# wubinzzu/NeuRec

Measured on NVIDIA H100. Metric: triplets/sec, higher is better.
Workload: dtype f32

## Files before the change

### include/neurec_b200.h

```cpp
#ifndef NEUREC_B200_H
#define NEUREC_B200_H

#include <stdint.h>

#ifdef __cplusplus
extern "C" {
#endif

#define NRC_OK 0
#define NRC_E_VALUE (-1)
#define NRC_E_TYPE (-2)
#define NRC_E_NOTIMPL (-3)
#define NRC_E_CUDA (-4)
#define NRC_E_LIMIT (-5)

#define NRC_METRIC_PRECISION 1
#define NRC_METRIC_RECALL 2
#define NRC_METRIC_MAP 3
#define NRC_METRIC_NDCG 4
#define NRC_METRIC_MRR 5

#define NRC_LOSS_BPR 0
#define NRC_LOSS_HINGE 1
#define NRC_LOSS_SQUARE 2
// ... 123 lines not shown
                       uint64_t seed, uint64_t epoch, int32_t batch_size, int64_t first_step,
                       int64_t num_steps, int32_t loss_kind, float reg, int32_t opt_kind,
                       const float* hyper_host, float* adam_pows, float* grad_user,
                       float* grad_item, int32_t* touched_user, int32_t* touched_item,
                       float* slot0_user, float* slot1_user, float* slot0_item, float* slot1_item,
                       int32_t first_stamp, int32_t* ws_users, int32_t* ws_items, void* ws_third,
                       float* step_loss, void* stream);

int nrc_batch_randint_choice(int32_t high, const int64_t* out_indptr, int32_t n_rows,
                             int64_t total_out, int32_t replace, const int64_t* excl_indptr,
                             const int32_t* excl_indices, uint64_t seed, uint64_t stream_id,
                             int32_t* out, void* stream);


int nrc_mf_pairwise_grad(const float* user_table, const float* item_table, int32_t dim,
                         const int32_t* users, const int32_t* pos_items,
                         const int32_t* neg_items, int64_t batch, int32_t loss_kind, float reg,
                         float* grad_user, float* grad_item, int32_t* touched_user,
                         int32_t* touched_item, int32_t stamp, float* loss, void* stream);

int nrc_mf_pointwise_grad(const float* user_table, const float* item_table, int32_t dim,
                          const int32_t* users, const int32_t* items, const float* labels,
                          int64_t batch, int32_t loss_kind, float reg, float* grad_user,
                          float* grad_item, int32_t* touched_user, int32_t* touched_item,
                          int32_t stamp, float* loss, void* stream);

int nrc_opt_apply_rows(int32_t opt_kind, float* var, float* grad, float* slot0, float* slot1,
                       const int32_t* touched, int32_t stamp, int64_t rows, int32_t dim,
                       const float* hyper_host, void* stream);

int nrc_mf_bpr_sgd_fused(float* user_table, float* item_table, int32_t dim, const int32_t* users,
                         const int32_t* pos_items, const int32_t* neg_items, int64_t batch,
                         float lr, float reg, float* loss, void* stream);

int nrc_mf_bpr_sgd_sharded(float* const* user_shards, float* const* item_shards, int32_t world,
                           int32_t self_rank, int64_t users_per_shard, int64_t items_per_shard, int32_t dim,
                           const int32_t* users, const int32_t* pos_items, const int32_t* neg_items,
                           int64_t batch, float lr, float reg, float* loss, void* stream);
int nrc_mf_bpr_sgd_epoch(float* user_table, float* const* item_shards, int32_t world,
                         int32_t self_rank, int64_t items_per_shard, int32_t dim,
                         const int64_t* train_indptr, const int32_t* train_indices,
                         const int32_t* pos_users, const int32_t* pos_items, int64_t n_pos,
                         int32_t num_items, int32_t shuffle, uint64_t seed, uint64_t epoch,
                         int64_t first, int64_t count, float lr, float reg, float* loss,
                         void* stream);

int nrc_mf_bpr_sgd_epoch_hot(float* user_table, float* const* item_shards, int32_t world,
                             int32_t self_rank, int64_t items_per_shard, int32_t dim,
                             const int64_t* train_indptr, const int32_t* train_indices,
                             const int32_t* pos_users, const int32_t* pos_items, int64_t n_pos,
                             int32_t num_items, int32_t shuffle, uint64_t seed, uint64_t epoch,
                             int64_t first, int64_t count, float lr, float reg, float* loss,
                             float* hot, float* hot_delta, int32_t n_hot, void* stream);
int nrc_mf_hot_apply(float* hot, float* hot_delta, int64_t n_floats, void* stream);

int nrc_mf_last_routes(int32_t* out);


int nrc_mf_bpr_lazy_adam_epoch(float* user_table, float* user_m, float* user_v, float* item_table,
                               float* item_m, float* item_v, int32_t dim, const int64_t* train_indptr,
                               const int32_t* train_indices, const int32_t* pos_users,
                               const int32_t* pos_items, int64_t n_pos, int32_t num_items,
                               int32_t shuffle, uint64_t seed, uint64_t epoch, int64_t first,
                               int64_t count, float lr_t, float beta1, float beta2, float eps,
                               float reg, float* loss, void* stream);

int nrc_shard_alloc(int64_t nbytes, void** dev_ptr_out, void* handle64_out);
int nrc_shard_free(void* dev_ptr);

int nrc_enable_peer_access(int32_t peer_device);
int nrc_ipc_export(const void* dev_ptr, void* handle64_out, int64_t* offset_out);
int nrc_ipc_open(const void* handle64, int64_t offset, void** dev_ptr_out);
int nrc_ipc_close(void* dev_ptr, int64_t offset);

int nrc_opt_apply_multi(int32_t opt_kind, int32_t n_vars, float* const* var, float* const* grad,
                        float* const* slot0, float* const* slot1, const int32_t* const* touched,
                        const int64_t* rows, const int32_t* dims, const int32_t* dense_var,
                        int32_t stamp, const float* hyper_host, void* stream);

int nrc_mf_train_epoch(float* user_table, float* item_table, int32_t num_users,
                       int32_t num_items, int32_t dim, const int32_t* users,
                       const int32_t* items, const void* third, int64_t n, int32_t batch_size,
                       int32_t pairwise, int32_t loss_kind, float reg, int32_t opt_kind,
                       const float* lr_t_host, const float* hyper_host, float* grad_user,
                       float* grad_item, int32_t* touched_user, int32_t* touched_item,
                       float* slot0_user, float* slot1_user, float* slot0_item,
                       float* slot1_item, int32_t first_stamp, float* step_loss, void* stream);

int nrc_mf_train_step_host(float* user_table, float* item_table, int32_t num_users,
                           int32_t num_items, int32_t dim, const int32_t* users_host,
                           const int32_t* items_host, const void* third_host, int64_t batch,
                           int32_t pairwise, int32_t loss_kind, float reg, int32_t opt_kind,
                           const float* hyper_host, float* grad_user, float* grad_item,
                           int32_t* touched_user, int32_t* touched_item, float* slot0_user,
                           float* slot1_user, float* slot0_item, float* slot1_item,
                           int32_t stamp, void* staging, float* loss_host, void* stream);


typedef struct nrc_ncf_shape {
    int32_t num_users, num_items;
    int32_t mf_dim, mlp_dim;
    int32_t n_layers;
    int32_t layers[4];
    int32_t n_towers;
} nrc_ncf_shape;

// ... 199 lines not shown
```

### neurec_b200/csrc/train_mf.cu

```cuda
#include <stdlib.h>

#include "common.cuh"
#include "epoch.cuh"
#include "learner.cuh"
#include "mf.cuh"
#include "mf_routes.cuh"
#include "optim.cuh"

namespace nrc {

int32_t g_mf_routes[kMfKernels][kMfFields] = {{-1, -1, -1, -1, -1, -1, -1}, {-1, -1, -1, -1, -1, -1, -1},
                                              {-1, -1, -1, -1, -1, -1, -1}, {-1, -1, -1, -1, -1, -1, -1},
                                              {-1, -1, -1, -1, -1, -1, -1}, {-1, -1, -1, -1, -1, -1, -1}};

template <bool PAIRWISE>
__global__ void __launch_bounds__(256)
mf_grad_kernel(const float* __restrict__ U, const float* __restrict__ V, int D, const int32_t* __restrict__ users,
               const int32_t* __restrict__ items, const int32_t* __restrict__ third, int64_t batch, int loss_kind,
               float reg, float* __restrict__ gU, float* __restrict__ gV, int32_t* __restrict__ tU,
               int32_t* __restrict__ tV, int32_t stamp, float* __restrict__ loss) {
    const int lane = threadIdx.x & 31;
    const int wib = threadIdx.x >> 5;
    const int wpb = blockDim.x >> 5;
    const float inv_b = 1.0f / (float)batch;
// ... 113 lines not shown
    mf_route(kMfSgdIds, dim == 128 ? 4 : dim == 64 ? 2 : 1, sharded, -1, -1, blocks, capped, -1);
    if (dim == 128) { if (sharded) NRC_LAUNCH_SGD(4, true); else NRC_LAUNCH_SGD(4, false); }
    else if (dim == 64) { if (sharded) NRC_LAUNCH_SGD(2, true); else NRC_LAUNCH_SGD(2, false); }
    else { if (sharded) NRC_LAUNCH_SGD(1, true); else NRC_LAUNCH_SGD(1, false); }
#undef NRC_LAUNCH_SGD
    NRC_CUDA_CHECK(cudaGetLastError());
    return NRC_OK;
}


template <int VEC>
constexpr int kSgdTierRows = 8192 / (32 * VEC);
template <int VEC>
constexpr size_t kSgdTierBytes = (size_t)2 * kSgdTierRows<VEC> * 32 * VEC * sizeof(float);

template <int VEC, bool SHARDED>
__device__ __forceinline__ void load_item(const RowShards& V, int32_t id, int nt, const float* s_val, int lane,
                                          float (&v)[VEC]) {
    if (id < nt) {
        ld_vec<VEC>(s_val + id * (32 * VEC) + lane * VEC, v);
    } else {
        bool remote;
        float* upd;
        ld_vec<VEC>(V.row<SHARDED>(id, 32 * VEC, remote, upd) + lane * VEC, v);
    }
}

template <int VEC, bool SHARDED>
__device__ __forceinline__ void update_item(const RowShards& V, int32_t id, int nt, float* s_dlt, int lane,
                                            const float (&d)[VEC]) {
    if (id < nt) {
#pragma unroll
        for (int t = 0; t < VEC; ++t) atomicAdd(s_dlt + id * (32 * VEC) + t * 32 + lane, d[t]);
    } else {
        bool remote;
        float* upd;
        V.row<SHARDED>(id, 32 * VEC, remote, upd);
        red_row<VEC>(upd + lane * VEC, d, remote && V.vec_remote == 0);
    }
}

__device__ __forceinline__ float add_as_red(float x, float d) {
    float r;
    asm("add.rn.ftz.f32 %0, %1, %2;" : "=f"(r) : "f"(x), "f"(d));
    return r;
}

constexpr int64_t kOnceMaxRow = 32;
constexpr int32_t kUserOnce = INT32_MIN;

__device__ __forceinline__ void stream_sample(const EpochSpec& E, int64_t p, int64_t first, int64_t count, bool user_once,
                                              int32_t& u, int32_t& item, int32_t& third) {
    const int64_t idx = feistel_perm(E.perm, p);
    u = __ldg(E.users + idx);
    item = __ldg(E.pos + idx);
    const int64_t beg = __ldg(E.tptr + u), end = __ldg(E.tptr + u + 1);
    third = philox_draw_excluding((uint64_t)(idx * E.neg_num), E.seed, E.stream_id, E.num_items, E.tidx + beg, end - beg);
    if (user_once && end - beg <= kOnceMaxRow) {
        bool alone = true;
#pragma unroll 1
        for (int64_t q = beg; q < end; ++q) {
            if (q == idx) continue;
            const int64_t r = feistel_perm_inv(E.perm, q);
            alone &= (uint64_t)(r - first) >= (uint64_t)count;
        }
        if (alone) u |= kUserOnce;
    }
}

constexpr int kStreamThreads = 768;

template <int VEC, bool SHARDED>
__global__ void __launch_bounds__(kStreamThreads, 1)
mf_bpr_sgd_stream_kernel(float* __restrict__ U_local, const RowShards V, const EpochSpec E, int64_t first,
                         int64_t count, int user_once, float lr, float reg, float* __restrict__ loss) {
    constexpr int D = 32 * VEC, CH = kStreamThreads, T = kSgdTierRows<VEC>;
    constexpr int TPW = 2;
    __shared__ int32_t s_u[CH], s_i[CH], s_j[CH];
    extern __shared__ __align__(16) float s_tier[];
    float* const s_val = s_tier;
    float* const s_dlt = s_tier + T * D;
    const int lane = threadIdx.x & 31, warp = threadIdx.x >> 5;
    const int nt = V.n_hot < T ? V.n_hot : T;
    for (int e = threadIdx.x; e < nt * D / 4; e += blockDim.x) {
        reinterpret_cast<float4*>(s_val)[e] = reinterpret_cast<const float4*>(V.hot)[e];
        reinterpret_cast<float4*>(s_dlt)[e] = make_float4(0.f, 0.f, 0.f, 0.f);
    }
    const int64_t lo = count * blockIdx.x / gridDim.x, hi = count * (blockIdx.x + 1) / gridDim.x;
    float loss_acc = 0.0f;
    for (int64_t c0 = lo; c0 < hi; c0 += CH) {
        const int n = (hi - c0 < CH) ? (int)(hi - c0) : CH;
        if ((int)threadIdx.x < n) {
            int32_t u, i, j;
            stream_sample(E, first + c0 + threadIdx.x, first, count, user_once != 0, u, i, j);
            s_u[threadIdx.x] = u; s_i[threadIdx.x] = i; s_j[threadIdx.x] = j;
        }
        __syncthreads();
        for (int t0 = warp * TPW; t0 < n; t0 += (kStreamThreads / 32) * TPW) {
            float a[TPW][VEC], b[TPW][VEC], c[TPW][VEC];
#pragma unroll
            for (int k = 0; k < TPW; ++k) {
                const int t = (t0 + k < n) ? t0 + k : t0;
                ld_vec<VEC>(U_local + (size_t)(s_u[t] & ~kUserOnce) * D + lane * VEC, a[k]);
                load_item<VEC, SHARDED>(V, s_i[t], nt, s_val, lane, b[k]);
                load_item<VEC, SHARDED>(V, s_j[t], nt, s_val, lane, c[k]);
            }
            float di[TPW], dj[TPW], sq[TPW];
#pragma unroll
            for (int k = 0; k < TPW; ++k) {
                di[k] = 0.f; dj[k] = 0.f; sq[k] = 0.f;
#pragma unroll
                for (int t = 0; t < VEC; ++t) {
                    di[k] = fmaf(a[k][t], b[k][t], di[k]); dj[k] = fmaf(a[k][t], c[k][t], dj[k]);
                    sq[k] += a[k][t] * a[k][t] + b[k][t] * b[k][t] + c[k][t] * c[k][t];
                }
                di[k] = warp_sum(di[k]); dj[k] = warp_sum(dj[k]);
            }
#pragma unroll
            for (int k = 0; k < TPW; ++k) {
                if (t0 + k >= n) break;
                const int t = t0 + k;
                const float x = di[k] - dj[k];
                float l = neg_log_sigmoid(x);
                if (reg != 0.0f) l += reg * 0.5f * warp_sum(sq[k]);
                loss_acc += l;
                const float g = neg_log_sigmoid_grad(x);
                float du[VEC], dvi[VEC], dvj[VEC];
#pragma unroll
                for (int q = 0; q < VEC; ++q) {
                    du[q] = -lr * (g * (b[k][q] - c[k][q]) + reg * a[k][q]);
                    dvi[q] = -lr * (g * a[k][q] + reg * b[k][q]);
                    dvj[q] = -lr * (-g * a[k][q] + reg * c[k][q]);
                }
                const int32_t su = s_u[t];
                float* const pu = U_local + (size_t)(su & ~kUserOnce) * D + lane * VEC;
                if (su & kUserOnce) {
#pragma unroll
                    for (int q = 0; q < VEC; ++q) du[q] = add_as_red(a[k][q], du[q]);
                    st_vec<VEC>(pu, du);
                } else {
                    red_row<VEC>(pu, du, false);
                }
                update_item<VEC, SHARDED>(V, s_i[t], nt, s_dlt, lane, dvi);
                update_item<VEC, SHARDED>(V, s_j[t], nt, s_dlt, lane, dvj);
            }
        }
        __syncthreads();
    }
    __syncthreads();
    for (int e = threadIdx.x; e < nt * 32; e += blockDim.x) {
        const int r = e >> 5, l = e & 31;
        float d[VEC];
        bool any = false;
#pragma unroll
        for (int t = 0; t < VEC; ++t) { d[t] = s_dlt[r * D + t * 32 + l]; any |= d[t] != 0.0f; }
        if (any) red_row<VEC>(V.hot_delta + (size_t)r * D + l * VEC, d, false);
    }
    if (lane == 0 && loss) atomicAdd(loss, loss_acc);
}

template <int VEC, bool SH>
static int launch_stream(float* U_local, const RowShards& SV, const EpochSpec& E, int64_t first, int64_t count,
                         int user_once, float lr, float reg, float* loss, cudaStream_t st) {
    constexpr size_t smem = kSgdTierBytes<VEC>;
    static int64_t grid_cap = 0;
    if (!grid_cap) {
        NRC_CUDA_CHECK(cudaFuncSetAttribute(mf_bpr_sgd_stream_kernel<VEC, SH>, cudaFuncAttributeMaxDynamicSharedMemorySize,
                                            (int)smem));
        int per_sm = 0;
        NRC_CUDA_CHECK(cudaOccupancyMaxActiveBlocksPerMultiprocessor(&per_sm, mf_bpr_sgd_stream_kernel<VEC, SH>, kStreamThreads, smem));
        NRC_REQUIRE(per_sm > 0, NRC_E_CUDA, "mf_bpr_sgd_stream_kernel does not fit on an SM");
        grid_cap = (int64_t)per_sm * sm_count();
    }
    int64_t blocks = (count + kStreamThreads - 1) / kStreamThreads;
    const bool capped = blocks > grid_cap;
    if (blocks > grid_cap) blocks = grid_cap;
    mf_route(kMfSgdCsr, VEC, SH, user_once, SV.n_hot < kSgdTierRows<VEC> ? SV.n_hot : kSgdTierRows<VEC>, blocks, capped,
             -1);
    mf_bpr_sgd_stream_kernel<VEC, SH><<<(unsigned)blocks, kStreamThreads, smem, st>>>(U_local, SV, E, first, count,
                                                                                      user_once, lr, reg, loss);
    NRC_CUDA_CHECK(cudaGetLastError());
    return NRC_OK;
}

static int launch_bpr_sgd_stream(float* U_local, const RowShards& SV, int dim, const EpochSpec& E, int64_t first,
                                 int64_t count, float lr, float reg, float* loss, cudaStream_t st) {
    const bool sharded = SV.rows_per_shard != 0;
    const int user_once = E.pos == E.tidx ? 1 : 0;
#define NRC_STREAM(VEC) (sharded ? launch_stream<VEC, true>(U_local, SV, E, first, count, user_once, lr, reg, loss, st) \
                                 : launch_stream<VEC, false>(U_local, SV, E, first, count, user_once, lr, reg, loss, st))
    if (dim == 128) return NRC_STREAM(4);
    if (dim == 64) return NRC_STREAM(2);
    return NRC_STREAM(1);
#undef NRC_STREAM
}

template <int VEC>
__device__ __forceinline__ void lazy_adam_row(float* var, float* m, float* v, const float (&x)[VEC], float (&mm)[VEC],
                                              float (&vv)[VEC], const float (&g)[VEC], float lr_t, float b1, float b2,
                                              float eps) {
    float out[VEC];
#pragma unroll
    for (int t = 0; t < VEC; ++t) {
        mm[t] = b1 * mm[t] + (1.0f - b1) * g[t];
        vv[t] = b2 * vv[t] + (1.0f - b2) * g[t] * g[t];
        out[t] = x[t] - lr_t * mm[t] / (sqrtf(vv[t]) + eps);
    }
    st_vec<VEC>(m, mm); st_vec<VEC>(v, vv); st_vec<VEC>(var, out);
}

template <int VEC>
__global__ void __launch_bounds__(256, 3)
mf_bpr_lazy_adam_stream_kernel(float* __restrict__ U, float* __restrict__ mU, float* __restrict__ vU, float* __restrict__ V,
                               float* __restrict__ mV, float* __restrict__ vV, const EpochSpec E, int64_t first, int64_t count,
                               float lr_t, float b1, float b2, float eps, float reg, float* __restrict__ loss) {
    constexpr int D = 32 * VEC;
    constexpr int CH = 256;
    __shared__ int32_t s_u[CH], s_i[CH], s_j[CH];
    const int lane = threadIdx.x & 31, warp = threadIdx.x >> 5;
    float loss_acc = 0.0f;
    for (int64_t c0 = (int64_t)blockIdx.x * CH; c0 < count; c0 += (int64_t)gridDim.x * CH) {
        const int n = (count - c0 < CH) ? (int)(count - c0) : CH;
        if ((int)threadIdx.x < n) {
            int32_t u, i, j;
            epoch_sample(E, first + c0 + threadIdx.x, 0, u, i, j);
            s_u[threadIdx.x] = u; s_i[threadIdx.x] = i; s_j[threadIdx.x] = j;
        }
        __syncthreads();
        for (int t = warp; t < n; t += 8) {
            const size_t ou = (size_t)s_u[t] * D + lane * VEC, oi = (size_t)s_i[t] * D + lane * VEC,
                         oj = (size_t)s_j[t] * D + lane * VEC;
            float a[VEC], bi[VEC], bj[VEC], mu[VEC], vu[VEC], mi[VEC], vi[VEC], mj[VEC], vj[VEC];
            ld_vec<VEC>(U + ou, a); ld_vec<VEC>(V + oi, bi); ld_vec<VEC>(V + oj, bj);
            ld_vec<VEC>(mU + ou, mu); ld_vec<VEC>(vU + ou, vu);
            ld_vec<VEC>(mV + oi, mi); ld_vec<VEC>(vV + oi, vi);
            ld_vec<VEC>(mV + oj, mj); ld_vec<VEC>(vV + oj, vj);
            float di = 0.f, dj = 0.f, sq = 0.f;
#pragma unroll
            for (int c = 0; c < VEC; ++c) {
                di = fmaf(a[c], bi[c], di); dj = fmaf(a[c], bj[c], dj);
                sq += a[c] * a[c] + bi[c] * bi[c] + bj[c] * bj[c];
            }
            di = warp_sum(di); dj = warp_sum(dj);
            const float x = di - dj;
            float l = neg_log_sigmoid(x);
            if (reg != 0.0f) l += reg * 0.5f * warp_sum(sq);
            loss_acc += l;
// ... 92 lines not shown
    if (batch <= 0) return NRC_OK;
    RowShards SU{}, SV{};
    for (int r = 0; r < world; ++r) {
        NRC_REQUIRE(user_shards[r] != nullptr && item_shards[r] != nullptr, NRC_E_VALUE, "shard %d is NULL", r);
        SU.base[r] = user_shards[r];
        SV.base[r] = item_shards[r];
    }
    SU.rows_per_shard = (int32_t)users_per_shard;
    SV.rows_per_shard = (int32_t)items_per_shard;
    SU.self = SV.self = self_rank;
    SU.vec_remote = SV.vec_remote = peer_red_mode();
    return launch_bpr_sgd(SU, SV, dim, users, pos_items, neg_items, batch, lr, reg, loss, as_stream(stream));
}

extern "C" int nrc_mf_bpr_sgd_epoch_hot(float* user_table, float* const* item_shards, int32_t world, int32_t self_rank,
                                    int64_t items_per_shard, int32_t dim, const int64_t* train_indptr,
                                    const int32_t* train_indices, const int32_t* pos_users, const int32_t* pos_items,
                                    int64_t n_pos, int32_t num_items, int32_t shuffle, uint64_t seed, uint64_t epoch,
                                    int64_t first, int64_t count, float lr, float reg, float* loss, float* hot, float* hot_delta,
                                    int32_t n_hot, void* stream) {
    NRC_REQUIRE(world >= 1 && world <= 8, NRC_E_LIMIT, "world %d outside [1, 8]", world);
    NRC_REQUIRE(self_rank >= 0 && self_rank < world, NRC_E_VALUE, "self_rank %d outside [0, %d)", self_rank, world);
    NRC_REQUIRE(user_table != nullptr && item_shards != nullptr, NRC_E_VALUE, "table pointers are NULL");
    NRC_REQUIRE(dim == 32 || dim == 64 || dim == 128, NRC_E_LIMIT, "fused SGD supports dim 32, 64, 128 (got %d)", dim);
    NRC_REQUIRE(world == 1 || (items_per_shard > 0 && items_per_shard * world < (1ll << 31) &&
                               items_per_shard * world >= num_items),
                NRC_E_VALUE, "items_per_shard %lld x world %d must cover num_items %d and fit int32",
                (long long)items_per_shard, world, num_items);
    EpochSpec E;
    int rc = epoch_spec_init(E, train_indptr, train_indices, pos_users, pos_items, n_pos, 1, num_items, 1, shuffle, seed,
                             epoch);
    if (rc) return rc;
    NRC_REQUIRE(first >= 0 && count >= 0 && first + count <= n_pos, NRC_E_VALUE,
                "[first, first + count) = [%lld, %lld) outside the epoch's %lld triplets", (long long)first,
                (long long)(first + count), (long long)n_pos);
    if (count == 0) return NRC_OK;
    RowShards SV{};
    for (int r = 0; r < world; ++r) {
        NRC_REQUIRE(item_shards[r] != nullptr, NRC_E_VALUE, "item shard %d is NULL", r);
        SV.base[r] = item_shards[r];
    }
    SV.rows_per_shard = world > 1 ? (int32_t)items_per_shard : 0;
    SV.self = self_rank;
    NRC_REQUIRE(n_hot >= 0 && n_hot <= num_items && (n_hot == 0 || (hot != nullptr && hot_delta != nullptr)), NRC_E_VALUE,
                "n_hot %d needs 0 <= n_hot <= num_items and the replica / delta buffers", n_hot);
    SV.hot = hot; SV.hot_delta = hot_delta; SV.n_hot = n_hot;
    {
        static int vec = -1, force = -1;
        if (vec < 0) vec = peer_red_mode();
        if (force < 0) { const char* e = getenv("NRC_FORCE_REMOTE_PATH"); force = e ? atoi(e) : 0; }
        SV.vec_remote = vec;
        SV.force_remote = force;
    }
    return launch_bpr_sgd_stream(user_table, SV, dim, E, first, count, lr, reg, loss, as_stream(stream));
}

extern "C" int nrc_mf_bpr_sgd_epoch(float* user_table, float* const* item_shards, int32_t world, int32_t self_rank,
                                    int64_t items_per_shard, int32_t dim, const int64_t* train_indptr,
                                    const int32_t* train_indices, const int32_t* pos_users, const int32_t* pos_items,
                                    int64_t n_pos, int32_t num_items, int32_t shuffle, uint64_t seed, uint64_t epoch,
                                    int64_t first, int64_t count, float lr, float reg, float* loss, void* stream) {
    return nrc_mf_bpr_sgd_epoch_hot(user_table, item_shards, world, self_rank, items_per_shard, dim, train_indptr,
                                    train_indices, pos_users, pos_items, n_pos, num_items, shuffle, seed, epoch, first,
                                    count, lr, reg, loss, nullptr, nullptr, 0, stream);
}

namespace nrc {
__global__ void __launch_bounds__(256) hot_apply_kernel(float4* __restrict__ hot, float4* __restrict__ delta, int64_t n4) {
    for (int64_t e = (int64_t)blockIdx.x * blockDim.x + threadIdx.x; e < n4; e += (int64_t)gridDim.x * blockDim.x) {
        float4 h = hot[e];
        const float4 d = delta[e];
        h.x += d.x; h.y += d.y; h.z += d.z; h.w += d.w;
        hot[e] = h;
        delta[e] = make_float4(0.f, 0.f, 0.f, 0.f);
    }
}
}

extern "C" int nrc_mf_hot_apply(float* hot, float* hot_delta, int64_t n_floats, void* stream) {
    NRC_REQUIRE(n_floats >= 0 && (n_floats & 3) == 0, NRC_E_VALUE, "n_floats %lld must be a multiple of 4", (long long)n_floats);
    if (n_floats == 0) return NRC_OK;
    NRC_REQUIRE(hot && hot_delta, NRC_E_VALUE, "replica / delta pointers are NULL");
    int64_t blocks = (n_floats / 4 + 255) / 256;
    const int64_t cap = (int64_t)sm_count() * 8;
    if (blocks > cap) blocks = cap;
    hot_apply_kernel<<<(unsigned)blocks, 256, 0, as_stream(stream)>>>(reinterpret_cast<float4*>(hot),
                                                                      reinterpret_cast<float4*>(hot_delta), n_floats / 4);
    NRC_CUDA_CHECK(cudaGetLastError());
    return NRC_OK;
}

extern "C" int nrc_mf_bpr_lazy_adam_epoch(float* user_table, float* user_m, float* user_v, float* item_table, float* item_m,
                                          float* item_v, int32_t dim, const int64_t* train_indptr,
                                          const int32_t* train_indices, const int32_t* pos_users, const int32_t* pos_items,
                                          int64_t n_pos, int32_t num_items, int32_t shuffle, uint64_t seed, uint64_t epoch,
                                          int64_t first, int64_t count, float lr_t, float beta1, float beta2, float eps,
                                          float reg, float* loss, void* stream) {
    NRC_REQUIRE(dim == 32 || dim == 64 || dim == 128, NRC_E_LIMIT, "lazy Adam supports dim 32, 64, 128 (got %d)", dim);
    NRC_REQUIRE(user_table && user_m && user_v && item_table && item_m && item_v, NRC_E_VALUE, "table / slot pointers are NULL");
    EpochSpec E;
    int rc = epoch_spec_init(E, train_indptr, train_indices, pos_users, pos_items, n_pos, 1, num_items, 1, shuffle, seed,
                             epoch);
    if (rc) return rc;
    NRC_REQUIRE(first >= 0 && count >= 0 && first + count <= n_pos, NRC_E_VALUE,
                "[first, first + count) = [%lld, %lld) outside the epoch's %lld triplets", (long long)first,
                (long long)(first + count), (long long)n_pos);
    if (count == 0) return NRC_OK;
// ... 149 lines not shown
```

Baseline: 850.1 million.

## Split CSR sampling into prefetched side-stream kernel and skip atomics for unique items

Triplet sampling moves out of the SGD stream kernel into a separate sampling kernel that writes u/i/j buffers. It also builds seen/multi bitmaps marking items that occur more than once in the window. The next window is sampled speculatively on a side stream, fenced by fork/join events, so it can overlap the SGD kernel of the current call. Items that appear only once in a window are updated with plain stores instead of reductions, and the user's CSR row bounds are inferred from a vectorised 16-wide load of the users array. The costs are extra buffers, memsets and bitmap atomics, host-side cache state keyed on the window, and a register cap of 64 on the SGD kernel.

```diff
diff --git a/include/neurec_b200.h b/include/neurec_b200.h
--- a/include/neurec_b200.h
+++ b/include/neurec_b200.h
@@ -199,6 +199,7 @@
                              int32_t num_items, int32_t shuffle, uint64_t seed, uint64_t epoch,
                              int64_t first, int64_t count, float lr, float reg, float* loss,
                              float* hot, float* hot_delta, int32_t n_hot, void* stream);
+int nrc_mf_sgd_prefetch(int32_t enable);
 int nrc_mf_hot_apply(float* hot, float* hot_delta, int64_t n_floats, void* stream);
 
 int nrc_mf_last_routes(int32_t* out);
diff --git a/neurec_b200/csrc/train_mf.cu b/neurec_b200/csrc/train_mf.cu
--- a/neurec_b200/csrc/train_mf.cu
+++ b/neurec_b200/csrc/train_mf.cu
@@ -189,9 +189,31 @@
 __device__ __forceinline__ void stream_sample(const EpochSpec& E, int64_t p, int64_t first, int64_t count, bool user_once,
                                               int32_t& u, int32_t& item, int32_t& third) {
     const int64_t idx = feistel_perm(E.perm, p);
-    u = __ldg(E.users + idx);
     item = __ldg(E.pos + idx);
-    const int64_t beg = __ldg(E.tptr + u), end = __ldg(E.tptr + u + 1);
+    int64_t beg = -1, end = -1;
+    const int64_t b0 = idx & ~(int64_t)15;
+    if (user_once && ((uintptr_t)E.users & 63) == 0 && b0 + 16 <= E.n_pos) {
+        int32_t v[16];
+#pragma unroll
+        for (int t = 0; t < 4; ++t) {
+            const int4 q = __ldg(reinterpret_cast<const int4*>(E.users + b0) + t);
+            v[4 * t] = q.x; v[4 * t + 1] = q.y; v[4 * t + 2] = q.z; v[4 * t + 3] = q.w;
+        }
+        const int k = (int)(idx - b0);
+        u = v[0];
+#pragma unroll
+        for (int t = 1; t < 16; ++t) u = t == k ? v[t] : u;
+        int lo = 0, hi = 16;
+#pragma unroll
+        for (int t = 0; t < 16; ++t) {
+            if (t < k && v[t] != u) lo = t + 1;
+            if (t > k && v[t] != u && hi == 16) hi = t;
+        }
+        if ((lo > 0 || b0 == 0) && (hi < 16 || b0 + 16 == E.n_pos)) { beg = b0 + lo; end = b0 + hi; }
+    } else {
+        u = __ldg(E.users + idx);
+    }
+    if (beg < 0) { beg = __ldg(E.tptr + u); end = __ldg(E.tptr + u + 1); }
     third = philox_draw_excluding((uint64_t)(idx * E.neg_num), E.seed, E.stream_id, E.num_items, E.tidx + beg, end - beg);
     if (user_once && end - beg <= kOnceMaxRow) {
         bool alone = true;
@@ -205,12 +227,46 @@
     }
 }
 
+struct SgdIds {
+    int32_t* u;
+    int32_t* i;
+    int32_t* j;
+    uint32_t* seen;
+    uint32_t* multi;
+};
+
+__global__ void __launch_bounds__(256, 8)
+sgd_sample_kernel(const EpochSpec E, int64_t first, int64_t count, int user_once, int32_t n_hot, SgdIds ids) {
+    for (int64_t k = (int64_t)blockIdx.x * blockDim.x + threadIdx.x; k < count; k += (int64_t)gridDim.x * blockDim.x) {
+        int32_t u, i, j;
+        stream_sample(E, first + k, first, count, user_once != 0, u, i, j);
+        ids.u[k] = u; ids.i[k] = i; ids.j[k] = j;
+#pragma unroll
+        for (int r = 0; r < 2; ++r) {
+            const int32_t id = r ? j : i;
+            if (id < n_hot) continue;
+            const uint32_t bit = 1u << (id & 31);
+            if (atomicOr(ids.seen + (id >> 5), bit) & bit) atomicOr(ids.multi + (id >> 5), bit);
+        }
+    }
+}
+
+template <bool SHARDED>
+__device__ __forceinline__ bool item_once(const RowShards& V, const uint32_t* multi, int32_t id) {
+    if constexpr (SHARDED) {
+        return false;
+    } else {
+        if (id < V.n_hot || V.force_remote) return false;
+        return ((__ldg(multi + (id >> 5)) >> (id & 31)) & 1u) == 0;
+    }
+}
+
 constexpr int kStreamThreads = 768;
 
 template <int VEC, bool SHARDED>
-__global__ void __launch_bounds__(kStreamThreads, 1)
-mf_bpr_sgd_stream_kernel(float* __restrict__ U_local, const RowShards V, const EpochSpec E, int64_t first,
-                         int64_t count, int user_once, float lr, float reg, float* __restrict__ loss) {
+__global__ void __maxnreg__(64)
+mf_bpr_sgd_stream_kernel(float* __restrict__ U_local, const RowShards V, const SgdIds ids, int64_t count, float lr,
+                         float reg, float* __restrict__ loss) {
     constexpr int D = 32 * VEC, CH = kStreamThreads, T = kSgdTierRows<VEC>;
     constexpr int TPW = 2;
     __shared__ int32_t s_u[CH], s_i[CH], s_j[CH];
@@ -224,23 +280,29 @@
         reinterpret_cast<float4*>(s_dlt)[e] = make_float4(0.f, 0.f, 0.f, 0.f);
     }
     const int64_t lo = count * blockIdx.x / gridDim.x, hi = count * (blockIdx.x + 1) / gridDim.x;
+    int32_t nu = 0, ni = 0, nj = 0;
+    auto fetch = [&](int64_t c0) {
+        const int64_t k = c0 + threadIdx.x;
+        if (k < hi) { nu = __ldg(ids.u + k); ni = __ldg(ids.i + k); nj = __ldg(ids.j + k); }
+    };
+    fetch(lo);
     float loss_acc = 0.0f;
     for (int64_t c0 = lo; c0 < hi; c0 += CH) {
         const int n = (hi - c0 < CH) ? (int)(hi - c0) : CH;
-        if ((int)threadIdx.x < n) {
-            int32_t u, i, j;
-            stream_sample(E, first + c0 + threadIdx.x, first, count, user_once != 0, u, i, j);
-            s_u[threadIdx.x] = u; s_i[threadIdx.x] = i; s_j[threadIdx.x] = j;
-        }
+        if ((int)threadIdx.x < n) { s_u[threadIdx.x] = nu; s_i[threadIdx.x] = ni; s_j[threadIdx.x] = nj; }
         __syncthreads();
+        fetch(c0 + CH);
         for (int t0 = warp * TPW; t0 < n; t0 += (kStreamThreads / 32) * TPW) {
             float a[TPW][VEC], b[TPW][VEC], c[TPW][VEC];
+            bool oi[TPW], oj[TPW];
 #pragma unroll
             for (int k = 0; k < TPW; ++k) {
                 const int t = (t0 + k < n) ? t0 + k : t0;
                 ld_vec<VEC>(U_local + (size_t)(s_u[t] & ~kUserOnce) * D + lane * VEC, a[k]);
                 load_item<VEC, SHARDED>(V, s_i[t], nt, s_val, lane, b[k]);
                 load_item<VEC, SHARDED>(V, s_j[t], nt, s_val, lane, c[k]);
+                oi[k] = item_once<SHARDED>(V, ids.multi, s_i[t]);
+                oj[k] = item_once<SHARDED>(V, ids.multi, s_j[t]);
             }
             float di[TPW], dj[TPW], sq[TPW];
 #pragma unroll
@@ -278,8 +340,20 @@
                 } else {
                     red_row<VEC>(pu, du, false);
                 }
-                update_item<VEC, SHARDED>(V, s_i[t], nt, s_dlt, lane, dvi);
-                update_item<VEC, SHARDED>(V, s_j[t], nt, s_dlt, lane, dvj);
+                if (oi[k]) {
+#pragma unroll
+                    for (int q = 0; q < VEC; ++q) dvi[q] = add_as_red(b[k][q], dvi[q]);
+                    st_vec<VEC>(V.base[0] + (size_t)s_i[t] * D + lane * VEC, dvi);
+                } else {
+                    update_item<VEC, SHARDED>(V, s_i[t], nt, s_dlt, lane, dvi);
+                }
+                if (oj[k]) {
+#pragma unroll
+                    for (int q = 0; q < VEC; ++q) dvj[q] = add_as_red(c[k][q], dvj[q]);
+                    st_vec<VEC>(V.base[0] + (size_t)s_j[t] * D + lane * VEC, dvj);
+                } else {
+                    update_item<VEC, SHARDED>(V, s_j[t], nt, s_dlt, lane, dvj);
+                }
             }
         }
         __syncthreads();
@@ -296,9 +370,89 @@
     if (lane == 0 && loss) atomicAdd(loss, loss_acc);
 }
 
+struct SgdWindow {
+    const int64_t* tptr;
+    const int32_t* tidx;
+    const int32_t* users;
+    const int32_t* pos;
+    int64_t n_pos, first, count;
+    uint64_t seed, epoch;
+    int32_t num_items, shuffle, n_hot;
+    bool operator==(const SgdWindow& o) const {
+        return tptr == o.tptr && tidx == o.tidx && users == o.users && pos == o.pos && n_pos == o.n_pos &&
+               first == o.first && count == o.count && seed == o.seed && epoch == o.epoch && num_items == o.num_items &&
+               shuffle == o.shuffle && n_hot == o.n_hot;
+    }
+};
+
+struct SgdPrefetch {
+    static constexpr int kSlots = 3, kCapture = 2;
+    void* mem = nullptr;
+    int64_t cap_ids = 0, cap_words = 0;
+    SgdIds slot[kSlots] = {};
+    int spec = -1;
+    SgdWindow spec_key{};
+    int cur = 0;
+    cudaStream_t side = nullptr;
+    cudaEvent_t fork = nullptr, join = nullptr;
+    ~SgdPrefetch() {
+        if (mem) cudaFree(mem);
+        if (side) cudaStreamDestroy(side);
+        if (fork) cudaEventDestroy(fork);
+        if (join) cudaEventDestroy(join);
+    }
+};
+constexpr int kMaxDevices = 16;
+static SgdPrefetch g_prefetch[kMaxDevices];
+static int g_prefetch_on = 1;
+
+static int prefetch_reserve(SgdPrefetch& P, int64_t count, int32_t num_items, bool capturing) {
+    const int64_t words = ((int64_t)num_items + 31) / 32;
+    if (!P.side) {
+        NRC_CUDA_CHECK(cudaStreamCreateWithFlags(&P.side, cudaStreamNonBlocking));
+        NRC_CUDA_CHECK(cudaEventCreateWithFlags(&P.fork, cudaEventDisableTiming));
+        NRC_CUDA_CHECK(cudaEventCreateWithFlags(&P.join, cudaEventDisableTiming));
+    }
+    if (count <= P.cap_ids && words <= P.cap_words) return NRC_OK;
+    NRC_REQUIRE(!capturing, NRC_E_VALUE,
+                "the CSR-fed step's sample buffers must grow to %lld triplets and %d items: make one such call before "
+                "capturing it", (long long)count, num_items);
+    const int64_t ci = count > P.cap_ids ? count : P.cap_ids, cw = words > P.cap_words ? words : P.cap_words;
+    if (P.mem) {
+        NRC_CUDA_CHECK(cudaDeviceSynchronize());
+        NRC_CUDA_CHECK(cudaFree(P.mem));
+        P.mem = nullptr;
+    }
+    const size_t ids_b = ((size_t)ci * sizeof(int32_t) + 255) & ~(size_t)255, map_b = ((size_t)cw * 4 + 255) & ~(size_t)255;
+    NRC_CUDA_CHECK(cudaMalloc(&P.mem, SgdPrefetch::kSlots * (3 * ids_b + 2 * map_b)));
+    char* m = static_cast<char*>(P.mem);
+    for (int s = 0; s < SgdPrefetch::kSlots; ++s) {
+        P.slot[s].u = reinterpret_cast<int32_t*>(m); m += ids_b;
+        P.slot[s].i = reinterpret_cast<int32_t*>(m); m += ids_b;
+        P.slot[s].j = reinterpret_cast<int32_t*>(m); m += ids_b;
+        P.slot[s].seen = reinterpret_cast<uint32_t*>(m); m += map_b;
+        P.slot[s].multi = reinterpret_cast<uint32_t*>(m); m += map_b;
+    }
+    P.cap_ids = ci; P.cap_words = cw;
+    P.spec = -1;
+    return NRC_OK;
+}
+
+static int sample_window(const SgdIds& S, const EpochSpec& E, const SgdWindow& w, cudaStream_t st) {
+    const size_t map_b = (((size_t)w.num_items + 31) / 32) * 4;
+    NRC_CUDA_CHECK(cudaMemsetAsync(S.seen, 0, map_b, st));
+    NRC_CUDA_CHECK(cudaMemsetAsync(S.multi, 0, map_b, st));
+    int64_t blocks = (w.count + 255) / 256;
+    const int64_t cap = (int64_t)sm_count() * 8;
+    if (blocks > cap) blocks = cap;
+    sgd_sample_kernel<<<(unsigned)blocks, 256, 0, st>>>(E, w.first, w.count, E.pos == E.tidx ? 1 : 0, w.n_hot, S);
+    NRC_CUDA_CHECK(cudaGetLastError());
+    return NRC_OK;
+}
+
 template <int VEC, bool SH>
-static int launch_stream(float* U_local, const RowShards& SV, const EpochSpec& E, int64_t first, int64_t count,
-                         int user_once, float lr, float reg, float* loss, cudaStream_t st) {
+static int launch_stream(float* U_local, const RowShards& SV, const SgdIds& ids, int64_t count, int user_once, float lr,
+                         float reg, float* loss, cudaStream_t st) {
     constexpr size_t smem = kSgdTierBytes<VEC>;
     static int64_t grid_cap = 0;
     if (!grid_cap) {
@@ -314,22 +468,71 @@
     if (blocks > grid_cap) blocks = grid_cap;
     mf_route(kMfSgdCsr, VEC, SH, user_once, SV.n_hot < kSgdTierRows<VEC> ? SV.n_hot : kSgdTierRows<VEC>, blocks, capped,
              -1);
-    mf_bpr_sgd_stream_kernel<VEC, SH><<<(unsigned)blocks, kStreamThreads, smem, st>>>(U_local, SV, E, first, count,
-                                                                                      user_once, lr, reg, loss);
+    mf_bpr_sgd_stream_kernel<VEC, SH><<<(unsigned)blocks, kStreamThreads, smem, st>>>(U_local, SV, ids, count, lr, reg,
+                                                                                      loss);
     NRC_CUDA_CHECK(cudaGetLastError());
     return NRC_OK;
 }
 
-static int launch_bpr_sgd_stream(float* U_local, const RowShards& SV, int dim, const EpochSpec& E, int64_t first,
-                                 int64_t count, float lr, float reg, float* loss, cudaStream_t st) {
+static int launch_bpr_sgd_stream(float* U_local, const RowShards& SV, int dim, const EpochSpec& E, const SgdWindow& w,
+                                 float lr, float reg, float* loss, cudaStream_t st) {
     const bool sharded = SV.rows_per_shard != 0;
     const int user_once = E.pos == E.tidx ? 1 : 0;
-#define NRC_STREAM(VEC) (sharded ? launch_stream<VEC, true>(U_local, SV, E, first, count, user_once, lr, reg, loss, st) \
-                                 : launch_stream<VEC, false>(U_local, SV, E, first, count, user_once, lr, reg, loss, st))
-    if (dim == 128) return NRC_STREAM(4);
-    if (dim == 64) return NRC_STREAM(2);
-    return NRC_STREAM(1);
+    int dev = 0;
+    NRC_CUDA_CHECK(cudaGetDevice(&dev));
+    NRC_REQUIRE(dev < kMaxDevices, NRC_E_LIMIT, "device %d beyond the %d the CSR-fed step keeps buffers for", dev,
+                kMaxDevices);
+    SgdPrefetch& P = g_prefetch[dev];
+    cudaStreamCaptureStatus cs = cudaStreamCaptureStatusNone;
+    NRC_CUDA_CHECK(cudaStreamIsCapturing(st, &cs));
+    const bool capturing = cs != cudaStreamCaptureStatusNone;
+    int rc = prefetch_reserve(P, w.count, w.num_items, capturing);
+    if (rc) return rc;
+    int use;
+    if (capturing) {
+        use = SgdPrefetch::kCapture;
+    } else if (P.spec >= 0 && P.spec_key == w) {
+        use = P.spec;
+    } else {
+        use = 1 - P.cur;
+        if (P.spec == use) P.spec = -1;
+    }
+    if (use != P.spec || capturing) {
+        rc = sample_window(P.slot[use], E, w, st);
+        if (rc) return rc;
+    }
+    bool ahead = false;
+    EpochSpec En;
+    SgdWindow wn = w;
+    if (!capturing) {
+        P.cur = use;
+        P.spec = -1;
+        if (g_prefetch_on) {
+            wn.first = w.first + w.count;
+            if (wn.first + w.count > w.n_pos) { wn.first = 0; wn.epoch = w.epoch + 1; }
+            ahead = wn.count <= wn.n_pos &&
+                    epoch_spec_init(En, w.tptr, w.tidx, w.users, w.pos, w.n_pos, 1, w.num_items, 1, w.shuffle, w.seed,
+                                    wn.epoch) == NRC_OK;
+        }
+    }
+    if (ahead) {
+        NRC_CUDA_CHECK(cudaEventRecord(P.fork, st));
+        NRC_CUDA_CHECK(cudaStreamWaitEvent(P.side, P.fork, 0));
+    }
+#define NRC_STREAM(VEC) (sharded ? launch_stream<VEC, true>(U_local, SV, P.slot[use], w.count, user_once, lr, reg, loss, st) \
+                                 : launch_stream<VEC, false>(U_local, SV, P.slot[use], w.count, user_once, lr, reg, loss, st))
+    rc = dim == 128 ? NRC_STREAM(4) : dim == 64 ? NRC_STREAM(2) : NRC_STREAM(1);
 #undef NRC_STREAM
+    if (ahead) {
+        const int nxt = 1 - use;
+        const int rs = sample_window(P.slot[nxt], En, wn, P.side);
+        NRC_CUDA_CHECK(cudaEventRecord(P.join, P.side));
+        NRC_CUDA_CHECK(cudaStreamWaitEvent(st, P.join, 0));
+        if (rs) return rs;
+        P.spec = nxt;
+        P.spec_key = wn;
+    }
+    return rc;
 }
 
 template <int VEC>
@@ -528,7 +731,20 @@
         SV.vec_remote = vec;
         SV.force_remote = force;
     }
-    return launch_bpr_sgd_stream(user_table, SV, dim, E, first, count, lr, reg, loss, as_stream(stream));
+    SgdWindow w{};
+    w.tptr = train_indptr; w.tidx = train_indices; w.users = pos_users; w.pos = pos_items;
+    w.n_pos = n_pos; w.first = first; w.count = count; w.seed = seed; w.epoch = epoch;
+    w.num_items = num_items; w.shuffle = shuffle ? 1 : 0; w.n_hot = n_hot;
+    return launch_bpr_sgd_stream(user_table, SV, dim, E, w, lr, reg, loss, as_stream(stream));
+}
+
+extern "C" int nrc_mf_sgd_prefetch(int32_t enable) {
+    const int was = g_prefetch_on;
+    if (enable >= 0) {
+        g_prefetch_on = enable ? 1 : 0;
+        for (auto& P : g_prefetch) P.spec = -1;
+    }
+    return was;
 }
 
 extern "C" int nrc_mf_bpr_sgd_epoch(float* user_table, float* const* item_shards, int32_t world, int32_t self_rank,
diff --git a/profiles/prefetch_breakdown.py b/profiles/prefetch_breakdown.py
--- /dev/null
+++ b/profiles/prefetch_breakdown.py
@@ -0,0 +1,72 @@
+import argparse
+import json
+import os
+import subprocess
+import sys
+
+ROOT = os.path.dirname(os.path.dirname(os.path.abspath(__file__)))
+
+RUN = """
+import json, sys
+sys.path.insert(0, %(root)r)
+import bench
+from neurec_b200 import _lib
+if %(inline)r:
+    _lib.load().nrc_mf_sgd_prefetch(0)
+line = bench.measure_sharded(20, 5, 1, 0, [], with_cpu=False)
+r = line["roofline"]
+print(json.dumps({"ms_per_step": line["ms_per_step"], "launch_us": r["launch_us"], "launch_us_min": r["launch_us_min"],
+                  "launch_us_max": r["launch_us_max"], "sync_us": r["replicated_head"]["sync_us_mean"]}))
+"""
+
+PROFILE = """
+import json, sys
+sys.path.insert(0, %(root)r)
+import torch
+import bench
+from neurec_b200 import _lib
+if %(inline)r:
+    _lib.load().nrc_mf_sgd_prefetch(0)
+with torch.profiler.profile(activities=[torch.profiler.ProfilerActivity.CUDA]) as prof:
+    bench.measure_sharded(10, 3, 1, 0, [], with_cpu=False)
+out = {}
+for e in prof.key_averages():
+    for key in ("sgd_stream_kernel", "sgd_sample_kernel"):
+        if key in e.key:
+            out[key] = {"count": e.count, "mean_us": e.device_time_total / max(e.count, 1)}
+print(json.dumps(out))
+"""
+
+
+def run_py(code):
+    r = subprocess.run([sys.executable, "-c", code], capture_output=True, text=True)
+    if r.returncode:
+        raise RuntimeError(r.stderr[-4000:])
+    return json.loads(r.stdout.strip().splitlines()[-1])
+
+
+def main():
+    ap = argparse.ArgumentParser()
+    ap.add_argument("out")
+    ap.add_argument("--parent", default=None)
+    ap.add_argument("--rounds", type=int, default=2)
+    args = ap.parse_args()
+    runs = [("prefetch", ROOT, False), ("inline", ROOT, True)]
+    if args.parent:
+        runs.insert(0, ("parent", os.path.abspath(args.parent), False))
+    res = {name: [] for name, _, _ in runs}
+    for _ in range(args.rounds):
+        for name, root, inline in runs:
+            res[name].append(run_py(RUN % {"root": root, "inline": inline}))
+            print(name, json.dumps(res[name][-1]), flush=True)
+    for name, inline in (("inline", True), ("prefetch", False)):
+        res["kernels_" + name] = run_py(PROFILE % {"root": ROOT, "inline": inline})
+        print("kernels_" + name, json.dumps(res["kernels_" + name]), flush=True)
+    res["gpu"] = subprocess.run(["nvidia-smi", "--query-gpu=name,power.limit,clocks.max.sm", "--format=csv,noheader"],
+                                capture_output=True, text=True).stdout.strip()
+    with open(args.out, "w") as f:
+        json.dump(res, f, indent=1)
+
+
+if __name__ == "__main__":
+    main()
```

After: 889.8 million, median of 6. +4.7%, better.

## Replace static block chunking with per-warp dynamic work claiming via global atomic counter

Applied to the files above, without the earlier changes.

The stream SGD kernel no longer splits the triplet range statically per block and synchronises the whole block per 768-triplet chunk. Each warp now claims 32-triplet slices from a global atomic counter, prefetching its next claim, samples its own slice into a per-warp region of shared memory, and uses __syncwarp instead of __syncthreads. The aim is to remove block-wide barrier stalls and tail imbalance across CTAs. In exchange it adds global atomic contention and a self-resetting counter that assumes launches do not overlap. A profiling script that instruments phase timings is also added.

```diff
diff --git a/neurec_b200/csrc/train_mf.cu b/neurec_b200/csrc/train_mf.cu
--- a/neurec_b200/csrc/train_mf.cu
+++ b/neurec_b200/csrc/train_mf.cu
@@ -207,6 +207,9 @@
 
 constexpr int kStreamThreads = 768;
 
+__device__ unsigned long long g_stream_claimed;
+__device__ unsigned int g_stream_done;
+
 template <int VEC, bool SHARDED>
 __global__ void __launch_bounds__(kStreamThreads, 1)
 mf_bpr_sgd_stream_kernel(float* __restrict__ U_local, const RowShards V, const EpochSpec E, int64_t first,
@@ -223,24 +226,32 @@
         reinterpret_cast<float4*>(s_val)[e] = reinterpret_cast<const float4*>(V.hot)[e];
         reinterpret_cast<float4*>(s_dlt)[e] = make_float4(0.f, 0.f, 0.f, 0.f);
     }
-    const int64_t lo = count * blockIdx.x / gridDim.x, hi = count * (blockIdx.x + 1) / gridDim.x;
+    __syncthreads();
+    int32_t* const w_u = s_u + warp * 32;
+    int32_t* const w_i = s_i + warp * 32;
+    int32_t* const w_j = s_j + warp * 32;
     float loss_acc = 0.0f;
-    for (int64_t c0 = lo; c0 < hi; c0 += CH) {
-        const int n = (hi - c0 < CH) ? (int)(hi - c0) : CH;
-        if ((int)threadIdx.x < n) {
+    unsigned long long claim = 0;
+    if (lane == 0) claim = atomicAdd(&g_stream_claimed, 32ull);
+    for (;;) {
+        const int64_t c0 = (int64_t)__shfl_sync(0xffffffffu, claim, 0);
+        if (c0 >= count) break;
+        if (lane == 0) claim = atomicAdd(&g_stream_claimed, 32ull);
+        const int n = (count - c0 < 32) ? (int)(count - c0) : 32;
+        if (lane < n) {
             int32_t u, i, j;
-            stream_sample(E, first + c0 + threadIdx.x, first, count, user_once != 0, u, i, j);
-            s_u[threadIdx.x] = u; s_i[threadIdx.x] = i; s_j[threadIdx.x] = j;
-        }
-        __syncthreads();
-        for (int t0 = warp * TPW; t0 < n; t0 += (kStreamThreads / 32) * TPW) {
+            stream_sample(E, first + c0 + lane, first, count, user_once != 0, u, i, j);
+            w_u[lane] = u; w_i[lane] = i; w_j[lane] = j;
+        }
+        __syncwarp();
+        for (int t0 = 0; t0 < n; t0 += TPW) {
             float a[TPW][VEC], b[TPW][VEC], c[TPW][VEC];
 #pragma unroll
             for (int k = 0; k < TPW; ++k) {
                 const int t = (t0 + k < n) ? t0 + k : t0;
-                ld_vec<VEC>(U_local + (size_t)(s_u[t] & ~kUserOnce) * D + lane * VEC, a[k]);
-                load_item<VEC, SHARDED>(V, s_i[t], nt, s_val, lane, b[k]);
-                load_item<VEC, SHARDED>(V, s_j[t], nt, s_val, lane, c[k]);
+                ld_vec<VEC>(U_local + (size_t)(w_u[t] & ~kUserOnce) * D + lane * VEC, a[k]);
+                load_item<VEC, SHARDED>(V, w_i[t], nt, s_val, lane, b[k]);
+                load_item<VEC, SHARDED>(V, w_j[t], nt, s_val, lane, c[k]);
             }
             float di[TPW], dj[TPW], sq[TPW];
 #pragma unroll
@@ -269,7 +280,7 @@
                     dvi[q] = -lr * (g * a[k][q] + reg * b[k][q]);
                     dvj[q] = -lr * (-g * a[k][q] + reg * c[k][q]);
                 }
-                const int32_t su = s_u[t];
+                const int32_t su = w_u[t];
                 float* const pu = U_local + (size_t)(su & ~kUserOnce) * D + lane * VEC;
                 if (su & kUserOnce) {
 #pragma unroll
@@ -278,11 +289,11 @@
                 } else {
                     red_row<VEC>(pu, du, false);
                 }
-                update_item<VEC, SHARDED>(V, s_i[t], nt, s_dlt, lane, dvi);
-                update_item<VEC, SHARDED>(V, s_j[t], nt, s_dlt, lane, dvj);
+                update_item<VEC, SHARDED>(V, w_i[t], nt, s_dlt, lane, dvi);
+                update_item<VEC, SHARDED>(V, w_j[t], nt, s_dlt, lane, dvj);
             }
         }
-        __syncthreads();
+        __syncwarp();
     }
     __syncthreads();
     for (int e = threadIdx.x; e < nt * 32; e += blockDim.x) {
@@ -294,6 +305,10 @@
         if (any) red_row<VEC>(V.hot_delta + (size_t)r * D + l * VEC, d, false);
     }
     if (lane == 0 && loss) atomicAdd(loss, loss_acc);
+    if (threadIdx.x == 0 && atomicAdd(&g_stream_done, 1u) == gridDim.x - 1) {
+        atomicExch(&g_stream_claimed, 0ull);
+        atomicExch(&g_stream_done, 0u);
+    }
 }
 
 template <int VEC, bool SH>
diff --git a/profiles/stream_phases.py b/profiles/stream_phases.py
--- /dev/null
+++ b/profiles/stream_phases.py
@@ -0,0 +1,209 @@
+import argparse
+import json
+import os
+import shutil
+import subprocess
+import sys
+import tempfile
+
+ROOT = os.path.dirname(os.path.dirname(os.path.abspath(__file__)))
+FIELDS = ("t_start", "t_loop_end", "t_end", "tier", "sample", "chunk_barrier", "rows", "misc", "tail_barrier", "flush",
+          "cta", "slot")
+NF = len(FIELDS)
+WARPS = 24
+
+HELPERS = r"""
+__device__ unsigned long long* g_ph_buf;
+__device__ unsigned int g_ph_ticket, g_ph_cap;
+__device__ __forceinline__ unsigned long long ph_gtime() {
+    unsigned long long t;
+    asm volatile("mov.u64 %0, %%globaltimer;" : "=l"(t));
+    return t;
+}
+#define PH_MARK(acc) { const long long c_ = clock64(); acc += c_ - ph_c; ph_c = c_; }
+extern "C" int nrc_phase_buf(void* p, unsigned int cap) {
+    const unsigned int z = 0;
+    cudaMemcpyToSymbol(g_ph_buf, &p, sizeof(p));
+    cudaMemcpyToSymbol(g_ph_cap, &cap, sizeof(cap));
+    cudaMemcpyToSymbol(g_ph_ticket, &z, sizeof(z));
+    return (int)cudaDeviceSynchronize();
+}
+"""
+
+START = """    const unsigned long long ph_t0 = ph_gtime();
+    unsigned long long ph_loop_end = 0;
+    long long ph_c = clock64(), ph_tier = 0, ph_sample = 0, ph_bar = 0, ph_rows = 0, ph_misc = 0, ph_tail = 0, ph_flush = 0;
+"""
+
+END = """    PH_MARK(ph_flush);
+    const unsigned long long ph_end = ph_gtime();
+    __shared__ unsigned int ph_slot;
+    __syncthreads();
+    if (threadIdx.x == 0) ph_slot = atomicAdd(&g_ph_ticket, 1u);
+    __syncthreads();
+    if (g_ph_buf && lane == 0 && ph_slot < g_ph_cap) {
+        unsigned long long* r = g_ph_buf + ((size_t)ph_slot * %(warps)d + warp) * %(nf)d;
+        r[0] = ph_t0; r[1] = ph_loop_end; r[2] = ph_end; r[3] = ph_tier; r[4] = ph_sample; r[5] = ph_bar; r[6] = ph_rows;
+        r[7] = ph_misc; r[8] = ph_tail; r[9] = ph_flush; r[10] = blockIdx.x; r[11] = ph_slot;
+    }
+""" % {"warps": WARPS, "nf": NF}
+
+TAIL = ("    }\n    __syncthreads();\n    // the tier's",
+        "    }\n    PH_MARK(ph_misc);\n    ph_loop_end = ph_gtime();\n    __syncthreads();\n    PH_MARK(ph_tail);\n"
+        "    // the tier's")
+
+FORMS = {
+    "warp_slices": [
+        ("    for (;;) {\n", "    PH_MARK(ph_tier);\n    for (;;) {\n"),
+        ("        __syncwarp();\n        // TPW triplets", "        PH_MARK(ph_sample);\n        __syncwarp();\n        // TPW triplets"),
+        ("        __syncwarp();   // every lane", "        PH_MARK(ph_rows);\n        __syncwarp();   // every lane"),
+        TAIL,
+    ],
+    "chunked": [
+        ("    float loss_acc = 0.0f;\n    for (", "    float loss_acc = 0.0f;\n    PH_MARK(ph_tier);\n    for ("),
+        ("        }\n        __syncthreads();\n        // TPW triplets",
+         "        }\n        PH_MARK(ph_sample);\n        __syncthreads();\n        PH_MARK(ph_bar);\n        // TPW triplets"),
+        ("        __syncthreads();\n    }\n    __syncthreads();\n    // the tier's",
+         "        PH_MARK(ph_rows);\n        __syncthreads();\n        PH_MARK(ph_bar);\n    }\n    __syncthreads();\n"
+         "    // the tier's"),
+        TAIL,
+    ],
+}
+
+RUN = r"""
+import ctypes, json, sys
+sys.path.insert(0, %(root)r)
+import numpy as np, torch
+import bench
+from neurec_b200 import ops, _lib
+from neurec_b200.util import peer
+cfg, K, W = bench.ShardedCfg, 20, 5
+ptr, idx = bench.synth_shard_csr(cfg, 0, 1)
+T = bench.TrainData(ptr, idx)
+del ptr, idx
+g = torch.Generator(device="cuda").manual_seed(30)
+U = torch.empty((cfg.users_per_gpu, cfg.dim), device="cuda").normal_(0, 0.01, generator=g)
+VS = peer.single(torch.empty((cfg.items_per_gpu, cfg.dim), device="cuda"))
+VS.local.normal_(0, 0.01, generator=g)
+VS.enable_hot(bench.n_hot_of(cfg, 1))
+ni, bs = cfg.items_per_gpu, cfg.batch
+spe = T.n_pos // bs
+loss = torch.zeros(1, device="cuda")
+grid = torch.cuda.get_device_properties(0).multi_processor_count
+cap = (K + 1) * grid
+buf = torch.zeros(cap * %(warps)d * %(nf)d, dtype=torch.int64, device="cuda")
+lib = _lib.load()
+state = {"g": 0}
+def step(ev=None):
+    e, s = divmod(state["g"], spe)
+    if ev: ev[0].record()
+    ops.mf_bpr_sgd_epoch(U, VS, T.ptr, T.idx, T.users, T.idx, ni, True, bench.SEED, e, s * bs, bs, cfg.lr, 0.0, loss)
+    if ev: ev[1].record()
+    VS.sync_hot()
+    state["g"] += 1
+for _ in range(W):
+    step()
+evs = [[torch.cuda.Event(enable_timing=True) for _ in range(2)] for _ in range(K)]
+torch.cuda.synchronize()
+assert lib.nrc_phase_buf(ctypes.c_void_p(buf.data_ptr()), ctypes.c_uint(cap)) == 0
+for k in range(K):
+    step(evs[k])
+torch.cuda.synchronize()
+np.save(%(raw)r, buf.view(cap, %(warps)d, %(nf)d).cpu().numpy())
+print(json.dumps({"grid": grid, "launch_us": [a.elapsed_time(b) * 1e3 for a, b in evs]}))
+"""
+
+
+def instrument(src):
+    a = src.index("mf_bpr_sgd_stream_kernel(float*")
+    b = src.index("template <int VEC, bool SH>\nstatic int launch_stream")
+    anchor = "    const int lane = threadIdx.x & 31, warp = threadIdx.x >> 5;\n"
+    fin = "    if (lane == 0 && loss) atomicAdd(loss, loss_acc);\n"
+    for form, patches in FORMS.items():
+        k = src[a:b]
+        for old, new in patches + [(anchor, anchor + START), (fin, END + fin)]:
+            if k.count(old) != 1:
+                break
+            k = k.replace(old, new)
+        else:
+            break
+    else:
+        raise SystemExit("mf_bpr_sgd_stream_kernel has the text of neither known form")
+    head = src[:a]
+    t = head.rindex("template <int VEC, bool SHARDED>")
+    return form, head[:t] + HELPERS + head[t:] + k + src[b:]
+
+
+def build_copy(root, work):
+    for d in ("neurec_b200", "include"):
+        shutil.copytree(os.path.join(root, d), os.path.join(work, d), copy_function=shutil.copy2,
+                        ignore=shutil.ignore_patterns("__pycache__", "*.so"))
+    shutil.copy2(os.path.join(root, "bench.py"), work)
+    path = os.path.join(work, "neurec_b200", "csrc", "train_mf.cu")
+    form, src = instrument(open(path).read())
+    with open(path, "w") as f:
+        f.write(src)
+    subprocess.run([sys.executable, "-c", "import sys; sys.path.insert(0, %r); from neurec_b200 import _build; _build.build()"
+                    % work], check=True)
+    return form
+
+
+def summarize(raw, grid, form):
+    import numpy as np
+    recs = raw[raw[:, 0, 2] > 0]
+    launch = recs[:, 0, 11] // grid
+    cyc = recs[:, :, 3:10].astype(np.float64)
+    tot = cyc.sum()
+    share = {FIELDS[3 + i]: float(cyc[:, :, i].sum() / tot) for i in range(7)}
+    spread_loop, spread_end, span, cta_loop_us = [], [], [], []
+    for L in np.unique(launch):
+        r = recs[launch == L]
+        t0 = r[:, :, 0].min()
+        loop_end = r[:, :, 1].max(1)
+        end = r[:, :, 2].max(1)
+        spread_loop.append(float(loop_end.max() - loop_end.min()) / 1e3)
+        spread_end.append(float(end.max() - end.min()) / 1e3)
+        span.append(float(end.max() - t0) / 1e3)
+        cta_loop_us.append(float(np.median(loop_end - r[:, :, 0].min(1))) / 1e3)
+    med = lambda x: float(np.median(x))
+    return {"form": form, "launches": int(len(np.unique(launch))), "ctas_per_launch": grid,
+            "share_of_warp_cycles": share,
+            "sample_plus_barriers": share["sample"] + share["chunk_barrier"] + share["tail_barrier"],
+            "cta_loop_end_spread_us_median": med(spread_loop), "cta_finish_spread_us_median": med(spread_end),
+            "cta_loop_us_median": med(cta_loop_us), "launch_span_us_median": med(span)}
+
+
+def main():
+    ap = argparse.ArgumentParser()
+    ap.add_argument("out")
+    ap.add_argument("--root", default=ROOT)
+    ap.add_argument("--label", default="this tree")
+    args = ap.parse_args()
+    import numpy as np
+    work = tempfile.mkdtemp(prefix="stream_phases_")
+    try:
+        form = build_copy(os.path.abspath(args.root), work)
+        raw_path = os.path.join(work, "raw.npy")
+        r = subprocess.run([sys.executable, "-c", RUN % {"root": work, "warps": WARPS, "nf": NF, "raw": raw_path}],
+                           capture_output=True, text=True)
+        if r.returncode:
+            raise RuntimeError(r.stderr[-4000:])
+        run = json.loads(r.stdout.strip().splitlines()[-1])
+        res = summarize(np.load(raw_path), run["grid"], form)
+        res["launch_us_instrumented_mean"] = float(np.mean(run["launch_us"]))
+    finally:
+        shutil.rmtree(work, ignore_errors=True)
+    print(args.label, json.dumps(res), flush=True)
+    out = {}
+    if os.path.exists(args.out):
+        with open(args.out) as f:
+            out = json.load(f)
+    out["gpu"] = subprocess.run(["nvidia-smi", "--query-gpu=name,power.limit,clocks.max.sm", "--format=csv,noheader"],
+                                capture_output=True, text=True).stdout.strip()
+    out[args.label] = res
+    with open(args.out, "w") as f:
+        json.dump(out, f, indent=1)
+
+
+if __name__ == "__main__":
+    main()
```

After: 850.1 million before, 854.6 million after (median of 6 runs). No clear change (+0.5%).
